# igrega348/energy-equiv-lattice-gnn

Hardware: AMD Instinct MI355X
Metric: lattice-graphs/s (fwd+bwd), 4-layer EnergyEquivGNN, ~1k nodes/~4k edges, 1/2/4/8 GPU (higher is better)
Workload: dtype f32

## Files before the change

energy-equiv-lattice-gnn_amd/gnn/_lib.py:

```python
from __future__ import annotations

import ctypes
import os
from typing import Dict, Optional, Tuple

import torch

LIB_PATH = os.environ.get("EELG_LIB") or os.path.join(os.path.dirname(os.path.abspath(__file__)),
                                                      "libeelg.so")

_P = ctypes.c_void_p
_I = ctypes.c_int
_F = ctypes.c_float
_D = ctypes.c_double
_LL = ctypes.c_longlong

_SIGS = {
    "eelg_version": ([], ctypes.c_char_p),
    "eelg_last_error": ([], ctypes.c_char_p),
    "eelg_tp_find": ([ctypes.c_char_p], _I),
    "eelg_tp_info": ([_I, _P, _P], _I),
    "eelg_sc_find": ([ctypes.c_char_p], _I),
    "eelg_sc_info": ([_I, _P, _P], _I),
    "eelg_sc_outputs": ([_I, _P], _I),
# ... 29 lines not shown
    "eelg_cgc_fwd": ([_P, _P, _P, _P, _P, _P, _I, _I, _P, _P], _I),
    "eelg_cgc_bwd": ([_P, _P, _P, _P, _P, _P, _I, _I, _P, _P, _P, _P], _I),
    "eelg_cgc_fwd_ef": ([_P, _P, _P, _P, _P, _P, _P, _P, _I, _I, _P, _P], _I),
    "eelg_cgc_fwd_ef_res": ([_P] * 6 + [_P, _I, _I, _P, _P, _P], _I),
    "eelg_cgc_bwd_ef": ([_P, _P, _P, _P, _P, _P, _P, _P, _I, _I, _P, _P, _P, _P, _P], _I),
    "eelg_cgc_bwd_ef_parts": ([_I], _I),
    "eelg_nnconv_fwd": ([_P, _P, _P, _P, _P, _I, _I, _P, _P], _I),
    "eelg_nnconv_bwd_edge": ([_P, _P, _P, _P, _P, _P, _I, _I, _P, _P, _P, _P], _I),
    "eelg_nnconv_bwd_w_parts": ([_I, _I], _I),
    "eelg_nnconv_bwd_w": ([_P, _P, _P, _P, _P, _P, _I, _I, _P, _P, _P], _I),
    "eelg_csr_spmm": ([_P, _P, _P, _I, _P, _I, _I, _I, _P, _I, _I, _P], _I),
    "eelg_sc_fwd": ([_I, _P, _P, _I, _I, _P, _P], _I),
    "eelg_sc_bwd_x": ([_I, _P, _P, _P, _I, _I, _P, _P], _I),
    "eelg_sc_bwd_x_cm": ([_I, _P, _P, _P, _I, _I, _P, _P, _P, _P], _I),
    "eelg_sc_bwd_coef": ([_I, _P, _P, _I, _I, _I, _P, _P], _I),
    "eelg_sc_bwd_coef_parts": ([_I, _I, _I], _I),
    "eelg_sc_cmajor": ([_I, _I, _P, _I, _I, _P, _P], _I),
    "eelg_scg_fwd": ([_P, _P, _P, _I, _P, _I, _I, _P, _I, _P], _I),
    "eelg_scg_bwd_x": ([_P, _P, _P, _I, _P, _I, _P, _I, _I, _P, _P], _I),
    "eelg_scg_bwd_coef": ([_P, _P, _P, _I, _P, _I, _P, _I, _I, _P, _P], _I),
    "eelg_linear_fwd": ([_P, _I, _P, _P, _I, _P, _I, _P, _P], _I),
    "eelg_linear_fwd_res": ([_P, _I, _P, _P, _P, _I, _P, _I, _P, _P], _I),
    "eelg_linear_bwd_w": ([_P, _I, _P, _I, _I, _I, _P, _I, _I, _P, _P], _I),
    "eelg_linear_bwd_w_x6": ([_P, _I, _P, _I, _I, _I, _I, _I, _P, _P], _I),
    "eelg_radial_plan": ([_I, _I, _P, _P], _I),
    "eelg_linear_pack_size": ([_P], ctypes.c_longlong),
    "eelg_linear_pack": ([_P, _P, _P, _P], _I),
    "eelg_linear_fwd_pk": ([_P, _I, _P, _P, _P, _I, _P, _I, _P, _P], _I),
    "eelg_split_bf16x3": ([_P, ctypes.c_longlong, _P, _P], _I),
    "eelg_sum_rows_work": ([_I, ctypes.c_longlong], ctypes.c_longlong),
    "eelg_sum_rows": ([_P, ctypes.c_longlong, _I, ctypes.c_longlong, ctypes.c_float, _P, _P,
                       ctypes.c_longlong, _P], _I),
    "eelg_radial_fwd": ([_P, _I, _P, _P, _I, _P, _P, _P], _I),
    "eelg_radial_bwd_chain": ([_P, _I, _I, _P, _P, _P, _P, _P, _P, _P, _P], _I),
    "eelg_radial_bwd_chain_rows": ([_P, _I, _I, _P, _I, _P, _P, _P, _P, _P, _P, _P, _P, _P], _I),
    "eelg_radial_bwd": ([_P, _I, _I, _P, _P, _P, _P, _P, _P, _P, _P], _I),
    "eelg_tp_bwd_sh": ([_I, _P, _P, _P, _P, _P, _I, _P, _F, _P, _P], _I),
    "eelg_radial_bwd_x": ([_P, _I, _P, _P, _P, _P], _I),
    "eelg_radial_bwd_gh": ([_P, _I, _I, _P, _P, _P, _P], _I),
    "eelg_edge_embed_bwd": ([_P, _P, _P, _P, _P, _I, _I, _I, _F, _F, _P, _I, _P, _P, _P, _P], _I),
    "eelg_batch_assemble": ([_P, _P, _P, _I, _I, _I, _P, _P], _I),
    "eelg_mandel_rotate": ([_P, _I, _P, _P, _I, _P, _P], _I),
    "eelg_stiffness_metrics": ([_P, _P, _P, _I, _I, _F, _P, _P], _I),
    "eelg_elastic_props": ([_P, _P, _I, _I, _P, _P, _P, _P], _I),
    "eelg_elastic_props_bwd": ([_P, _P, _P, _P, _P, _P, _I, _I, _P, _P], _I),
    "eelg_transverse_props": ([_P, _P, _I, _I, _P, _P, _P, _P, _P, _P], _I),
    "eelg_transverse_props_bwd": ([_P, _P, _P, _P, _P, _P, _I, _I, _P, _P], _I),
    "eelg_stiffness_loss": ([_P, _P, _I, _I, _F, _P, _P, _P], _I),
    "eelg_sqnorm_parts": ([_LL], _I),
    "eelg_grad_sqnorm": ([_P, _LL, _P, _P], _I),
    "eelg_adamw_flat": ([_P, _P, _P, _P, _P, _LL, _P, _D, _D, _D, _D, _D, _D, _I, _P, _P, _P], _I),
    "eelg_strut_volume": ([_P] * 9 + [_I, _I, _I, _P, _P], _I),
    "eelg_design_step": ([_P] * 16 + [_I, _I, _I] + [_F] * 6 + [_I, _P, _P, _P], _I),
}

LIN_MAXSRC, LIN_MAXSLOT, LINW_MAXINS = 4, 8, 8


class LinSrc(ctypes.Structure):
    _fields_ = [("x_off", _I), ("k", _I), ("w_off", _I), ("ldk", _I), ("ldj", _I), ("alpha", _F)]


class LinSlot(ctypes.Structure):
    _fields_ = [("y_off", _I), ("n_out", _I), ("d", _I), ("bias_off", _I), ("n_src", _I),
                ("src", LinSrc * LIN_MAXSRC), ("r_off", _I)]


class LinDesc(ctypes.Structure):
    _fields_ = [("n_slots", _I), ("max_jt", _I), ("max_rows", _I), ("res_row", _I),
                ("slot", LinSlot * LIN_MAXSLOT)]


class LinWIns(ctypes.Structure):
    _fields_ = [("x_off", _I), ("k", _I), ("g_off", _I), ("n_out", _I), ("d", _I), ("w_off", _I),
                ("alpha", _F), ("ldw", _I)]


class LinWDesc(ctypes.Structure):
    _fields_ = [("n_ins", _I), ("max_jt", _I), ("max_ut", _I), ("max_rows", _I),
                ("ins", LinWIns * LINW_MAXINS)]

BATCH_MAXW = 64
METRICS_COLS = 16
ELASTIC_COLS = 12
TRANSVERSE_COLS = 7
TRANSVERSE_DIR_COLS = 5
OPTIM_STATE_COLS = 4
DESIGN_THREADS = 256


class BatchSrc(ctypes.Structure):
    _fields_ = [(k, _P) for k in ("positions", "node_attrs", "rowend", "srowend", "sender", "receiver",
                                  "shifts", "edge_attr", "perm", "sperm")] + \
               [(k, _I) for k in ("node_w", "edge_w", "total_nodes", "total_edges")]


class BatchOut(ctypes.Structure):
    _fields_ = [(k, _P) for k in ("positions", "node_attrs", "batch", "ptr", "rowptr", "srowptr",
                                  "edge_index", "shifts", "edge_attr", "perm", "sperm", "sender",
                                  "receiver")]


RADIAL_MAXH = 3
GATE_MAXBLK = 8
CGC_MAXD = 256
NNC_WIDTHS = (32, 64)
GATE_MAXGATED = 2048
GATE_MAXGATES = 512


class GateDesc(ctypes.Structure):
    _fields_ = [("n_scal", _I), ("n_gates", _I), ("n_blk", _I), ("pad", _I),
                ("blk_mul", _I * GATE_MAXBLK), ("blk_dim", _I * GATE_MAXBLK)]


SCG_MAXD = 25
SCG_CHUNK = 256


class ScgDesc(ctypes.Structure):
    _fields_ = [("D", _I), ("Dout", _I), ("mul", _I), ("nterms", _I),
                ("xb", _I * SCG_MAXD), ("xs", _I * SCG_MAXD), ("ob", _I * SCG_MAXD),
                ("os", _I * SCG_MAXD), ("orow", _I * (SCG_MAXD + 1))]


class RadialDesc(ctypes.Structure):
    _fields_ = [("n_feat", _I), ("hidden", _I), ("n_hidden", _I), ("n_out", _I),
                ("w", _P * RADIAL_MAXH), ("b", _P * RADIAL_MAXH)]


EXPORTED_SYMBOLS = tuple(_SIGS)

_lib = None


class EELGError(RuntimeError):
    pass


def load() -> ctypes.CDLL:
    global _lib
# ... 143 lines not shown
```

energy-equiv-lattice-gnn_amd/gnn/model.py:

```python
from __future__ import annotations

import os
from argparse import Namespace
from typing import Any, Dict

import torch

from . import ops
from .blocks import (Cart_4_to_Mandel, GeneralNonLinearReadoutBlock, MACELayer, PositiveLayer,
                     Spherical_to_Cartesian, as_csr)
from .irreps import Irreps
from .o3 import Linear


def storage_dtype(params: Namespace) -> torch.dtype:
    name = str(getattr(params, "storage_dtype", "float32")).replace("torch.", "")
    table = {"float32": torch.float32, "fp32": torch.float32, "bfloat16": torch.bfloat16,
             "bf16": torch.bfloat16}
    if name not in table:
        raise ValueError(f"storage_dtype {name!r}: expected 'float32' or 'bfloat16'")
    return table[name]


RADIAL_AHEAD_OF_LAYER1 = os.environ.get("EELG_RADIAL_BEFORE_L1", "1") != "0"
# ... 114 lines not shown
    def _radial_weights_ahead(self, edge_feats, csr=None, edge_sh=None):
        geom = torch.is_grad_enabled() and edge_feats.requires_grad
        if geom or not (ops.OVERLAP and edge_feats.is_cuda):
            return [None] * self.num_interactions, [None] * self.num_interactions
        main = torch.cuda.current_stream(edge_feats.device)
        side = ops.side_stream(edge_feats.device)
        side.wait_stream(main)
        edge_feats.record_stream(side)
        ws, evs = [], []
        with torch.cuda.stream(side):
            for layer in self.layers:
                smap = layer.interaction.strut_map(csr, edge_feats, edge_sh) if csr is not None else None
                w = layer.interaction.radial_weights(edge_feats, smap)
                ev = torch.cuda.Event()
                ev.record(side)
                ws.append(w)
                evs.append(ev)
        for w in ws:
            self._main_stream_weight(w).record_stream(main)
        return ws, evs

    @staticmethod
    def _main_stream_weight(w):
        return w.w if isinstance(w, ops.StrutWeights) else w

    def _coefficients_ahead(self, device) -> None:
        if not (ops.OVERLAP and COEF_AHEAD and device.type == "cuda"):
            return
        main = torch.cuda.current_stream(device)
        side = ops.side_stream(device, 1)
        side.wait_stream(main)
        for i, layer in enumerate(self.layers):
            layer.product.symmetric_contractions.coefficients_ahead(
                side, live=self.live_pruned and i == self.num_interactions - 1)

    def forward(self, edge_index, node_ft, edge_sh, edge_feats, batch_idx, num_graphs: int):
        csr, edge_sh, edge_feats = as_csr(edge_index, node_ft.shape[0], edge_sh, edge_feats)
        ws, evs = self._radial_weights_ahead(edge_feats, csr, edge_sh)
        self._coefficients_ahead(node_ft.device)

        def run(i, h, residual=None):
            if evs[i] is not None:
                torch.cuda.current_stream(h.device).wait_event(evs[i])
            live = self.live_pruned and i == self.num_interactions - 1
            return self.layers[i](h, csr, edge_sh, edge_feats, tp_weights=ws[i], residual=residual,
                                  live=live)

        node_ft = run(0, node_ft)
        if RADIAL_AHEAD_OF_LAYER1 and evs[-1] is not None:
            torch.cuda.current_stream(node_ft.device).wait_event(evs[-1])
        for i in range(1, self.num_interactions):
            node_ft = run(i, node_ft, residual=node_ft)
        out = self.nonlin_readout(node_ft, live=self.live_pruned)
        graph_ft = ops.graph_pool(out, batch_idx, num_graphs, self.global_reduction)
        stiff = self.sph_to_cart(self.linear(graph_ft, live=self.live_pruned))
        return self.positive_layer(self.cart_to_Mandel(stiff))


class _Embed1(torch.autograd.Function):

    @staticmethod
    def forward(ctx, attrs, weight, bias):
        ctx.save_for_backward(attrs)
        ctx.has_bias = bias is not None
        w = weight[:, 0]
        return torch.addcmul(bias, attrs, w) if bias is not None else attrs * w

    @staticmethod
    def backward(ctx, gy):
        from . import ops
        (attrs,) = ctx.saved_tensors
        gy = ops._f32(gy).contiguous()
        gw = ops.sum_rows(gy * attrs).unsqueeze(1) if ctx.needs_input_grad[1] else None
        gb = ops.sum_rows(gy) if ctx.has_bias and ctx.needs_input_grad[2] else None
        return None, gw, gb


def _embed(lin: torch.nn.Linear, attrs: torch.Tensor) -> torch.Tensor:
    if lin.in_features != 1:
        return lin(attrs)
    if attrs.is_cuda and not attrs.requires_grad:
        return _Embed1.apply(attrs, lin.weight, lin.bias)
    return torch.addcmul(lin.bias, attrs, lin.weight[:, 0]) if lin.bias is not None \
        else attrs * lin.weight[:, 0]


def _geometry_key(batch, n_edges: int):
    ts = [getattr(batch, k, None) for k in ("positions", "shifts", "edge_attr")]
    if not all(torch.is_tensor(t) for t in ts) or any(t.requires_grad for t in ts):
        return None
    pos, shifts, radius = ts
    if radius.numel() != n_edges or tuple(shifts.shape) != (n_edges, 3) or pos.dim() != 2 or pos.shape[1] != 3:
        return None
    return tuple((t.data_ptr(), t._version, tuple(t.shape), str(t.device)) for t in ts)


class EnergyEquivGNN(torch.nn.Module):
    def __init__(self, params: Namespace, *args: Any, **kwargs: Any) -> None:
        super().__init__(*args, **kwargs)
        self.params = params
        hidden = Irreps(params.hidden_irreps)
        self.node_ft_embedding = torch.nn.Linear(1, hidden.count("0e"))
        self.number_of_edge_basis = params.num_edge_bases
        self.max_edge_radius = params.max_edge_radius
        self.lmax = params.lmax
        self.stiffness_head = GNN_Head(params)

    @staticmethod
    def edge_graph(batch, strut: bool = True, build: bool = True) -> ops.EdgeCSR:
        n = batch.node_attrs.shape[0]
        ei = batch.edge_index
        dev = ei.device
        key = (ei.data_ptr(), ei._version, tuple(ei.shape), n, str(dev))
        csr = getattr(batch, "_eelg_csr", None)
        if csr is None or getattr(batch, "_eelg_csr_key", None) != key:
            pre = getattr(batch, "csr", None)
            if isinstance(pre, dict) and torch.is_tensor(pre.get("perm")):
                csr = ops.EdgeCSR.from_dict({k: (v.to(dev) if torch.is_tensor(v) else v)
                                             for k, v in pre.items()}, n)
            else:
                csr = ops.EdgeCSR.build(batch.edge_index, n)
            try:
                batch._eelg_csr = csr
                batch._eelg_csr_key = key
            except AttributeError:
                pass
        geo_key = _geometry_key(batch, csr.num_edges) if strut and ops.STRUT_WEIGHTS else None
        if geo_key is None:
            return csr
        if csr.strut is not None and getattr(csr, "_strut_key", None) != geo_key:
            csr.strut = None
        if csr.strut is None and build:
            csr.strut = ops.build_strut_map(batch.positions, csr.sender, csr.receiver,
                                            batch.shifts[csr.perm], batch.edge_attr[csr.perm].reshape(-1))
            csr._strut_key = geo_key
        return csr

    def forward(self, batch) -> Dict[str, torch.Tensor]:
        dev = batch.positions.device
        if dev.type != "cuda":
            raise RuntimeError("the EnergyEquivGNN hot path runs only on a HIP device "
                               "(got a CPU batch); move the model and batch to 'cuda'")
        with torch.cuda.device(dev):
            return self._forward(batch)

    def _forward(self, batch) -> Dict[str, torch.Tensor]:
        csr = self.edge_graph(batch, build=False)
        node_ft = _embed(self.node_ft_embedding, batch.node_attrs)
        geom = torch.is_grad_enabled() and (batch.positions.requires_grad or batch.shifts.requires_grad
                                            or batch.edge_attr.requires_grad)
        if geom and storage_dtype(self.params) != torch.float32:
            raise NotImplementedError(
                "geometry gradients (positions / shifts / edge_attr requiring grad) are built for "
                "fp32 storage only, not storage_dtype='bfloat16'")
        shifts = ops.permute_rows(batch.shifts, csr.perm)
        radius = ops.permute_rows(batch.edge_attr, csr.perm).reshape(-1)
        edge_sh, edge_feats = ops.edge_embed(batch.positions, csr, shifts, radius, self.lmax,
                                             self.number_of_edge_basis, 0.6, self.max_edge_radius)
        c = self.stiffness_head(csr, node_ft, edge_sh, edge_feats, batch.batch, batch.num_graphs)
        return {"stiffness": c}
```

energy-equiv-lattice-gnn_amd/gnn/ops.py:

```python
from __future__ import annotations

import contextlib
import ctypes
import math
import os
import weakref
from dataclasses import dataclass
from typing import Dict, Optional

import torch

from . import _lib


KernelTimer, TIMER, _launch = _lib.KernelTimer, _lib.TIMER, _lib.launch

OVERLAP = os.environ.get("EELG_OVERLAP", "1") != "0"
LIVE_OUT = os.environ.get("EELG_LIVE_OUT", "1") != "0"
SC_CMAJOR_ON_SIDE = os.environ.get("EELG_SC_CMAJOR_SIDE", "0") != "0"
SC_COEF_ON_SIDE = os.environ.get("EELG_SC_COEF_SIDE", "1") != "0"
RADIAL_CHAIN = os.environ.get("EELG_RADIAL_CHAIN", "1") != "0"
_TBS = os.environ.get("EELG_TP_BWD_SENDER", "0")
TP_BWD_SENDER = None if _TBS == "auto" else _TBS != "0"
TP_BWD_SPOS = os.environ.get("EELG_TP_BWD_SPOS", "0") != "0"
# ... 47 lines not shown
    def rep_rows(self, feats: torch.Tensor) -> torch.Tensor:
        memo = getattr(self, "_rep_rows", None)
        if memo is not None and memo[0]() is feats and memo[1] == feats._version:
            return memo[2]
        rows = feats[self.rep]
        self._rep_rows = (weakref.ref(feats), feats._version, rows)
        return rows


def _key_bits(v: torch.Tensor) -> torch.Tensor:
    return (v + 0.0).contiguous().view(torch.int32).to(torch.int64)


def build_strut_map(pos: torch.Tensor, sender: torch.Tensor, receiver: torch.Tensor,
                    shifts_sorted: torch.Tensor, radius_sorted: torch.Tensor) -> StrutMap:
    e = int(sender.shape[0])
    dev = sender.device
    ar = torch.arange(e, device=dev)
    if e == 0:
        z = torch.zeros(0, device=dev, dtype=torch.int64)
        return StrutMap(z, z.to(torch.int32), z, 0)
    s, r = sender.long(), receiver.long()
    pos = pos.detach().to(torch.float32)
    vec = (pos[r] - pos[s]) + shifts_sorted.detach().to(torch.float32)
    rad = _key_bits(radius_sorted.detach().to(torch.float32).reshape(e, 1))
    fwd = torch.cat([s[:, None], r[:, None], _key_bits(vec), rad], 1)
    rev = torch.cat([r[:, None], s[:, None], _key_bits(-vec), rad], 1)
    _, inv = torch.unique(torch.cat([fwd, rev]), dim=0, return_inverse=True)
    kf, kr = inv[:e], inv[e:]
    nk = int(inv.max()) + 1
    cnt = torch.zeros(nk, device=dev, dtype=torch.int64).index_add_(0, kf, torch.ones_like(kf))
    owner = torch.full((nk,), -1, device=dev, dtype=torch.int64)
    owner[kf] = ar
    cand = owner[kr]
    ok = (cnt[kf] == 1) & (cnt[kr] == 1) & (cand >= 0)
    partner = torch.where(ok, cand, ar)
    is_rep = partner >= ar
    rep = torch.nonzero(is_rep).reshape(-1)
    row_of = torch.cumsum(is_rep.to(torch.int64), 0) - 1
    row = row_of[torch.minimum(partner, ar)].to(torch.int32)
    return StrutMap(partner, row.contiguous(), rep, int(rep.shape[0]))


@dataclass
class EdgeCSR:
    perm: torch.Tensor
    sender: torch.Tensor
    receiver: torch.Tensor
    rowptr: torch.Tensor
    sperm: torch.Tensor
    srowptr: torch.Tensor
    num_nodes: int
    strut: Optional[StrutMap] = None

    @property
    def num_edges(self) -> int:
        return int(self.sender.shape[0])

    def sender_pos(self) -> torch.Tensor:
        sp = getattr(self, "_spos", None)
        if sp is None:
            sp = torch.empty_like(self.sperm)
            sp[self.sperm.long()] = torch.arange(self.sperm.shape[0], device=self.sperm.device,
                                                 dtype=self.sperm.dtype)
            self._spos = sp
        return sp

    @staticmethod
    def from_dict(d: Dict, num_nodes: int) -> "EdgeCSR":
        return EdgeCSR(d["perm"], d["sender"], d["receiver"], d["rowptr"], d["sperm"],
                       d["srowptr"], num_nodes)

    @staticmethod
    def build(edge_index: torch.Tensor, num_nodes: int) -> "EdgeCSR":
        from .data import build_edge_csr
        return EdgeCSR.from_dict(build_edge_csr(edge_index, num_nodes), num_nodes)


def edge_embed(pos, csr: EdgeCSR, shifts_sorted, radius_sorted, lmax: int, nb: int,
               len_end: float, rad_end: float):
    _require_device(pos, shifts_sorted, radius_sorted)
    if torch.is_grad_enabled() and (pos.requires_grad or shifts_sorted.requires_grad
                                    or radius_sorted.requires_grad):
        return _EdgeEmbed.apply(pos, shifts_sorted, radius_sorted, csr, lmax, nb, float(len_end),
                                float(rad_end))
    return _edge_embed_fwd(pos, csr, shifts_sorted, radius_sorted, lmax, nb, len_end, rad_end)


def _edge_embed_fwd(pos, csr: EdgeCSR, shifts_sorted, radius_sorted, lmax: int, nb: int,
                    len_end: float, rad_end: float):
    e = csr.num_edges
    nsh = (lmax + 1) ** 2
    sh = torch.empty(e, sh_row_stride(nsh), device=pos.device, dtype=torch.float32)
    feats = torch.empty(e, 2 * nb, device=pos.device, dtype=torch.float32)
    _launch("edge_embed", _lib.load().eelg_edge_embed, _f32(pos), csr.sender, csr.receiver,
            _f32(shifts_sorted), _f32(radius_sorted), e, lmax, nb, float(len_end), float(rad_end),
            sh, feats, on=sh)
    return sh[:, :nsh], feats


class _EdgeEmbed(torch.autograd.Function):

    @staticmethod
    def forward(ctx, pos, shifts_sorted, radius_sorted, csr: EdgeCSR, lmax, nb, len_end, rad_end):
        pos, shifts_sorted, radius_sorted = _f32(pos), _f32(shifts_sorted), _f32(radius_sorted)
        ctx.save_for_backward(pos, shifts_sorted, radius_sorted)
# ... 64 lines not shown
def padded_sh(sh: torch.Tensor) -> torch.Tensor:
    nsh = sh.shape[1]
    nshp = sh_row_stride(nsh)
    if (sh.dtype == torch.float32 and sh.stride() == (nshp, 1) and sh.storage_offset() == 0
            and sh.untyped_storage().nbytes() >= sh.shape[0] * nshp * 4):
        return sh
    out = torch.zeros(sh.shape[0], nshp, device=sh.device, dtype=torch.float32)
    out[:, :nsh] = sh
    return out[:, :nsh]


def segment_sum_csr(src, rowptr, n_rows: int, idx=None, row_scale=None, scale: float = 1.0):
    _require_device(src)
    bf = src.dtype == torch.bfloat16
    src = src.contiguous() if bf else _f32(src)
    width = src[0].numel() if src.shape[0] > 0 else int(torch.tensor(src.shape[1:]).prod())
    out = torch.empty((n_rows,) + tuple(src.shape[1:]), device=src.device, dtype=torch.float32)
    lib = _lib.load()
    fn = lib.eelg_segment_sum_csr_bf16 if bf else lib.eelg_segment_sum_csr
    _launch("segment_sum_csr", fn, src, rowptr, idx, row_scale, float(scale), n_rows, int(width), out,
            on=out)
    return out


def segment_sum_long(src: torch.Tensor, rowptr: torch.Tensor, n_rows: int,
                     row_scale: Optional[torch.Tensor] = None, scale: float = 1.0) -> torch.Tensor:
    _require_device(src)
    src = _f32(src)
    width = src.shape[1]
    n_split = max(1, min(64, -(-2048 // max(n_rows, 1))))
    work = torch.empty(n_rows, n_split, width, device=src.device, dtype=torch.float32)
    out = torch.empty(n_rows, width, device=src.device, dtype=torch.float32)
    _launch("segment_sum_split", _lib.load().eelg_segment_sum_split, src, rowptr, None, row_scale,
            float(scale), n_rows, width, n_split, work, out, on=out, timed="segment_sum_split")
    return out


class _SegmentMean(torch.autograd.Function):

    @staticmethod
    def forward(ctx, src, ptr32, batch, inv_cnt):
        ctx.save_for_backward(batch, inv_cnt)
        n_rows = ptr32.shape[0] - 1
        if src.shape[0] >= 64 * max(n_rows, 1):
            return segment_sum_long(src, ptr32, n_rows, row_scale=inv_cnt)
        return segment_sum_csr(src, ptr32, n_rows, row_scale=inv_cnt)

    @staticmethod
    def backward(ctx, g):
        batch, inv_cnt = ctx.saved_tensors
        return (g * inv_cnt[:, None])[batch], None, None, None


def graph_pool(src, batch, num_graphs: int, reduce: str = "mean"):
    _require_device(src)
    bounds = torch.arange(num_graphs + 1, device=batch.device, dtype=batch.dtype)
    ptr = torch.searchsorted(batch, bounds).to(torch.int32)
    cnt = (ptr[1:] - ptr[:-1]).to(torch.int64)
    if reduce == "mean":
        inv = 1.0 / cnt.clamp_min(1).to(torch.float32)
    elif reduce in ("sum", "add"):
        inv = torch.ones(num_graphs, device=src.device, dtype=torch.float32)
    elif reduce in ("max", "min", "mul"):
        return segment_pool_order(src, ptr, num_graphs, reduce)
    else:
        raise ValueError(f"global_reduction {reduce!r} not supported "
                         "(torch_scatter reduces: sum, add, mean, max, min, mul)")
    return _SegmentMean.apply(src, ptr, batch, inv)


_ORDER_OPS = {"max": 0, "min": 1, "mul": 2}


class _SegmentOrder(torch.autograd.Function):

    @staticmethod
    def forward(ctx, src, rowptr, n_rows: int, op: int, covered: bool):
        src = _f32(src)
        width = src.shape[1]
        out = torch.empty(n_rows, width, device=src.device, dtype=torch.float32)
        arg = (torch.empty(n_rows, width, device=src.device, dtype=torch.int32)
               if op != _ORDER_OPS["mul"] else None)
        _launch("segment_order", _lib.load().eelg_segment_order, src, rowptr, n_rows, width, op, out,
                arg, on=out)
        ctx.save_for_backward(src, rowptr, arg)
        ctx.n_rows, ctx.op, ctx.covered = n_rows, op, covered
        return out

    @staticmethod
    def backward(ctx, g):
        src, rowptr, arg = ctx.saved_tensors
        g = _f32(g)
        gs = torch.empty_like(src) if ctx.covered else torch.zeros_like(src)
        _launch("segment_order_bwd", _lib.load().eelg_segment_order_bwd, src, rowptr, arg, g,
                ctx.n_rows, src.shape[1], ctx.op, gs, on=gs)
        return gs, None, None, None, None


def segment_order(src, rowptr32, n_rows: int, reduce: str, covered: bool = False):
    _require_device(src)
    if reduce not in _ORDER_OPS:
        raise ValueError(f"segment_order: reduce {reduce!r} (max, min, mul)")
    return _SegmentOrder.apply(src, rowptr32, n_rows, _ORDER_OPS[reduce], covered)


def segment_pool_order(src, ptr32, num_graphs: int, reduce: str):
    return segment_order(src, ptr32, num_graphs, reduce)


PNA_FUSED = os.environ.get("EELG_PNA_FUSED", "1") != "0"
PNA_EPS = 1e-5


# ... 926 lines not shown
        g = _f32(g)
        sp, mul = ctx.sp, ctx.mul
        nt, nk = sp.shape
        a, t = sp.on(g.device)
        gt = g.t().contiguous()
        gw = torch.empty(nk, mul, device=g.device, dtype=torch.float32)
        _spmm(t, nk, gt, mul, 1, mul, gw, mul, 1)
        return gw, None, None


def symcon_coefficients(w: torch.Tensor, sp: SparseRows, ld: Optional[int] = None) -> torch.Tensor:
    return _SymConCoef.apply(w, sp, sp.shape[0] if ld is None else ld)


LOSS_FUSED = os.environ.get("EELG_LOSS_FUSED", "1") != "0"


class _StiffnessLoss(torch.autograd.Function):
    @staticmethod
    def forward(ctx, pred, target, grad_scale: float):
        _require_device(pred, target)
        nb = int(target.shape[0])
        p2 = _f32(pred).reshape(nb, -1)
        t2 = _f32(target).reshape(nb, -1)
        n = int(t2.shape[1])
        out = torch.empty(2, device=pred.device, dtype=torch.float32)
        grad = torch.empty_like(p2)
        with torch.cuda.device(pred.device):
            _launch("stiffness_loss", _lib.load().eelg_stiffness_loss, p2, t2, nb, n,
                    float(grad_scale), out, grad, on=pred, timed="stiffness_loss")
        ctx.save_for_backward(grad)
        ctx.shape = pred.shape
        loss, mean = out[0], out[1]
        ctx.mark_non_differentiable(mean)
        return loss, mean

    @staticmethod
    def backward(ctx, g_loss, g_mean):
        (grad,) = ctx.saved_tensors
        return (grad * g_loss).view(ctx.shape), None, None


def stiffness_loss_fused(pred: torch.Tensor, target: torch.Tensor, grad_scale: float = 1.0):
    if tuple(pred.shape) != tuple(target.shape) or pred.dim() < 2:
        raise ValueError(f"stiffness_loss_fused: pred {tuple(pred.shape)}, target {tuple(target.shape)}")
    if LOSS_FUSED and pred.is_cuda:
        return _StiffnessLoss.apply(pred, target.detach(), float(grad_scale))
    dims = tuple(range(1, target.dim()))
    per_graph = torch.nn.functional.mse_loss(pred, target, reduction="none").mean(dim=dims)
    loss = 100 * (per_graph / target.pow(2).mean(dim=dims)).mean()
    if grad_scale != 1.0:
        loss = loss.detach() + (loss - loss.detach()) * grad_scale
    return loss, per_graph.detach().mean()
```

include/eelg.h:

```cpp
#ifndef EELG_H
#define EELG_H

#include <stdint.h>

#ifdef __cplusplus
extern "C" {
#endif

const char* eelg_version(void);
const char* eelg_last_error(void);

int eelg_tp_find(const char* name);
int eelg_tp_info(int cfg, int* info7, uint64_t* sig);
int eelg_sc_find(const char* name);
int eelg_sc_info(int cfg, int* info8, uint64_t* sig);
int eelg_sc_outputs(int cfg, int* ls8);
int eelg_sc_find_outputs(int cfg, const int* ls, int n_ls);

int eelg_edge_embed(const float* pos, const int* sender, const int* receiver, const float* shifts,
                    const float* radius, int n_edges, int lmax, int nb, float len_end,
                    float rad_end, float* sh, float* feats, void* stream);

int eelg_tp_fwd(int cfg, const float* x, const float* sh, const float* w, const int* sender,
                const int* rowptr, int n_nodes, float inv_norm, float* agg, void* stream);
// ... 237 lines not shown
  int64_t* edge_index; float* shifts; float* edge_attr; int64_t* perm; int* sperm; int* sender;
  int* receiver;
} eelg_batch_out;
int eelg_batch_assemble(const eelg_batch_src* src, const int* table, const float* rot, int n_graphs,
                        int n_nodes, int n_edges, const eelg_batch_out* out, void* stream);

int eelg_mandel_rotate(const float* src, int n_src, const int* sel, const float* rot, int n_graphs,
                       float* out, void* stream);

#define EELG_METRICS_COLS 16
int eelg_stiffness_metrics(const float* pred, const float* target, const float* dirs, int n_graphs,
                           int n_dirs, float scale, float* out, void* stream);

#define EELG_ELASTIC_COLS 12
int eelg_elastic_props(const float* c, const float* dirs, int n_graphs, int n_dirs, float* props,
                       float* e_dir, float* s, void* stream);
int eelg_elastic_props_bwd(const float* s, const float* dirs, const float* e_dir, const float* props,
                           const float* g_props, const float* g_e_dir, int n_graphs, int n_dirs,
                           float* g_c, void* stream);

#define EELG_TRANSVERSE_COLS 7
#define EELG_TRANSVERSE_DIR_COLS 5
int eelg_transverse_props(const float* c, const float* dirs, int n_graphs, int n_dirs, float* props,
                          float* t_dir, int* arg, float* n_ext, double* s, void* stream);
int eelg_transverse_props_bwd(const double* s, const float* dirs, const float* props, const int* arg,
                              const float* g_props, const float* g_t_dir, int n_graphs, int n_dirs,
                              float* g_c, void* stream);

#define EELG_SQNORM_CHUNK 8192
#define EELG_SQNORM_MAXPARTS 1024
#define EELG_OPTIM_STATE_COLS 4
int eelg_stiffness_loss(const float* pred, const float* target, int n_graphs, int n, float grad_scale,
                        float* out, float* grad, void* stream);
int eelg_sqnorm_parts(long long numel);
int eelg_grad_sqnorm(const float* grad, long long numel, float* partials, void* stream);
int eelg_adamw_flat(float* p, float* m, float* v, float* vmax, float* grad, long long numel,
                    const float* partials, double lr, double beta1, double beta2, double eps,
                    double weight_decay, double max_norm, int amsgrad, const int* state_in, int* state_out,
                    void* stream);

#define EELG_DESIGN_THREADS 256
int eelg_strut_volume(const float* pos, const float* r, const float* shifts, const int* send,
                      const int* recv, const int* node_ptr, const int* edge_ptr,
                      const int* node_ptr_host, const int* edge_ptr_host, int n_graphs, int n_nodes,
                      int n_edges, float* vol, void* stream);
int eelg_design_step(const float* g_pos, const float* g_r, float* pos, float* r, const float* pos0,
                     float* m_pos, float* m_r, const int* partner, const int* node_ptr,
                     const int* edge_ptr, const int* node_ptr_host, const int* edge_ptr_host,
                     const float* shifts, const int* send, const int* recv, const float* v0,
                     int n_graphs, int n_nodes, int n_edges, float step_r, float step_pos, float beta,
                     float r_min, float r_max, float move_limit, int keep_volume, float* vol, int* flag,
                     void* stream);

#ifdef __cplusplus
}
#endif
#endif
```

Measured before the change: 2342.

## Fuse stiffness head (linear, sph-to-cart, Mandel, positive map) into one kernel

Adds a HIP kernel that, per graph, applies the final equivariant linear, the spherical-to-Cartesian projection, the Mandel mapping and the positive matrix function in one block, with a matching backward kernel that computes per-graph input, weight and bias gradients and sums them afterwards. This replaces a chain of small per-op launches and autograd nodes at the end of the model. It also caches the graph-pool segment bounds on the CSR object so searchsorted is not redone every step. In exchange, the kernels do their arithmetic in double precision with one 64-thread block per graph, and the backward writes per-graph weight-gradient rows that need an extra reduction.

```diff
diff --git a/energy-equiv-lattice-gnn_amd/csrc/eelg_head.hip b/energy-equiv-lattice-gnn_amd/csrc/eelg_head.hip
--- /dev/null
+++ b/energy-equiv-lattice-gnn_amd/csrc/eelg_head.hip
@@ -0,0 +1,250 @@
+#include <hip/hip_runtime.h>
+#include <stdint.h>
+
+#include "../../include/eelg.h"
+#include "eelg_internal.h"
+
+#define HEAD_THREADS 64
+#define HEAD_Y 21
+#define HEAD_CART 81
+#define HEAD_C 36
+
+template <typename TI, typename TO>
+__device__ __forceinline__ void head_linear(const eelg_lin_desc& desc, const TI* __restrict__ in,
+                                            const float* __restrict__ w, const float* __restrict__ bias,
+                                            TO* __restrict__ out) {
+  int base = 0;
+  for (int s = 0; s < desc.n_slots; ++s) {
+    const eelg_lin_slot& sl = desc.slot[s];
+    const int d = sl.d, cols = sl.n_out * d;
+    for (int c = (int)threadIdx.x - base; c < cols; c += HEAD_THREADS) {
+      if (c < 0) continue;
+      const int j = c / d, m = c - j * d;
+      double acc = 0.0;
+      for (int t = 0; t < sl.n_src; ++t) {
+        const eelg_lin_src& src = sl.src[t];
+        const TI* __restrict__ xi = in + src.x_off + m;
+        const float* __restrict__ wj = w + src.w_off + (size_t)j * src.ldj;
+        for (int k = 0; k < src.k; ++k) acc = fma((double)xi[k * d], (double)(wj[(size_t)k * src.ldk] * src.alpha), acc);
+      }
+      if (bias && sl.bias_off >= 0) acc += (double)bias[sl.bias_off + j];
+      out[sl.y_off + c] = (TO)acc;
+    }
+    base = (base + cols) % HEAD_THREADS;
+  }
+}
+
+__device__ __forceinline__ double head_base(double a, int idx, int pos) {
+  const double eye = (idx / 6 == idx % 6) ? 1.0 : 0.0;
+  if (pos == EELG_HEAD_TRUNC_EXP_2) return eye + a / 2.0;
+  if (pos == EELG_HEAD_TRUNC_EXP_4) return eye + a / 4.0;
+  return a;
+}
+
+__device__ __forceinline__ double head_square(const double* m, int i, int j) {
+  double acc = 0.0;
+#pragma unroll
+  for (int k = 0; k < 6; ++k) acc = fma(m[i * 6 + k], m[k * 6 + j], acc);
+  return acc;
+}
+
+__device__ __forceinline__ double head_square_bwd(const double* g, const double* m, int i, int j) {
+  double acc = 0.0;
+#pragma unroll
+  for (int k = 0; k < 6; ++k) acc = fma(g[i * 6 + k], m[j * 6 + k], acc);
+#pragma unroll
+  for (int k = 0; k < 6; ++k) acc = fma(m[k * 6 + i], g[k * 6 + j], acc);
+  return acc;
+}
+
+__device__ __forceinline__ bool head_squares(int pos) { return pos != EELG_HEAD_NONE; }
+__device__ __forceinline__ bool head_fourth(int pos) {
+  return pos == EELG_HEAD_POWER_4 || pos == EELG_HEAD_TRUNC_EXP_4;
+}
+
+__global__ __launch_bounds__(HEAD_THREADS) void head_fwd_kernel(
+    const float* __restrict__ x, int x_row, const float* __restrict__ w, const float* __restrict__ bias,
+    eelg_lin_desc desc, const float* __restrict__ q, const float* __restrict__ map, int pos,
+    float* __restrict__ c_out, float* __restrict__ a_out) {
+  __shared__ double s_y[HEAD_Y], s_z[HEAD_CART], s_m[HEAD_C], s_s[HEAD_C];
+  const int b = blockIdx.x, tid = threadIdx.x;
+  if (tid < HEAD_Y) s_y[tid] = 0.0;
+  __syncthreads();
+  head_linear(desc, x + (size_t)b * x_row, w, bias, s_y);
+  __syncthreads();
+  for (int r = tid; r < HEAD_CART; r += HEAD_THREADS) {
+    double acc = 0.0;
+#pragma unroll
+    for (int i = 0; i < HEAD_Y; ++i) acc = fma(s_y[i], (double)q[i * HEAD_CART + r], acc);
+    s_z[r] = acc;
+  }
+  __syncthreads();
+  double a = 0.0;
+  if (tid < HEAD_C) {
+    for (int r = 0; r < HEAD_CART; ++r) a = fma(s_z[r], (double)map[r * HEAD_C + tid], a);
+    a_out[(size_t)b * HEAD_C + tid] = (float)a;
+    s_m[tid] = head_base(a, tid, pos);
+  }
+  __syncthreads();
+  double c = a;
+  if (head_squares(pos)) {
+    if (tid < HEAD_C) c = head_square(s_m, tid / 6, tid % 6);
+    if (head_fourth(pos)) {
+      if (tid < HEAD_C) s_s[tid] = c;
+      __syncthreads();
+      if (tid < HEAD_C) c = head_square(s_s, tid / 6, tid % 6);
+    }
+  }
+  if (tid < HEAD_C) c_out[(size_t)b * HEAD_C + tid] = (float)c;
+}
+
+__global__ __launch_bounds__(HEAD_THREADS) void head_bwd_kernel(
+    const float* __restrict__ g_c, const float* __restrict__ a_in, const float* __restrict__ x, int x_row,
+    const float* __restrict__ w, eelg_lin_desc fdesc, eelg_lin_desc xdesc, eelg_linw_desc wdesc,
+    const float* __restrict__ q, const float* __restrict__ map, int pos, int n_w, int n_b,
+    float* __restrict__ g_x, int gx_row, float* __restrict__ g_wb) {
+  extern __shared__ float s_w[];
+  __shared__ double s_y[HEAD_Y], s_z[HEAD_CART], s_m[HEAD_C], s_s[HEAD_C], s_g[HEAD_C], s_t[HEAD_C];
+  const int b = blockIdx.x, tid = threadIdx.x;
+  const int i6 = tid / 6, j6 = tid % 6;
+  for (int e = tid; e < n_w + n_b; e += HEAD_THREADS) s_w[e] = 0.f;
+  if (tid < HEAD_C) {
+    s_m[tid] = head_base((double)a_in[(size_t)b * HEAD_C + tid], tid, pos);
+    s_g[tid] = (double)g_c[(size_t)b * HEAD_C + tid];
+  }
+  __syncthreads();
+  if (head_squares(pos)) {
+    if (head_fourth(pos)) {
+      if (tid < HEAD_C) s_s[tid] = head_square(s_m, i6, j6);
+      __syncthreads();
+      if (tid < HEAD_C) s_t[tid] = head_square_bwd(s_g, s_s, i6, j6);
+      __syncthreads();
+      if (tid < HEAD_C) s_g[tid] = s_t[tid];
+      __syncthreads();
+    }
+    double ga = 0.0;
+    if (tid < HEAD_C) {
+      ga = head_square_bwd(s_g, s_m, i6, j6);
+      if (pos == EELG_HEAD_TRUNC_EXP_2) ga = ga / 2.0;
+      if (pos == EELG_HEAD_TRUNC_EXP_4) ga = ga / 4.0;
+    }
+    __syncthreads();
+    if (tid < HEAD_C) s_g[tid] = ga;
+    __syncthreads();
+  }
+  for (int r = tid; r < HEAD_CART; r += HEAD_THREADS) {
+    double acc = 0.0;
+#pragma unroll
+    for (int c = 0; c < HEAD_C; ++c) acc = fma((double)map[r * HEAD_C + c], s_g[c], acc);
+    s_z[r] = acc;
+  }
+  __syncthreads();
+  if (tid < HEAD_Y) {
+    double acc = 0.0;
+    for (int r = 0; r < HEAD_CART; ++r) acc = fma((double)q[tid * HEAD_CART + r], s_z[r], acc);
+    s_y[tid] = acc;
+  }
+  __syncthreads();
+  head_linear(xdesc, s_y, w, nullptr, g_x + (size_t)b * gx_row);
+  const float* __restrict__ xb = x + (size_t)b * x_row;
+  for (int t = 0; t < wdesc.n_ins; ++t) {
+    const eelg_linw_ins& in = wdesc.ins[t];
+    const int ldw = in.ldw ? in.ldw : in.n_out;
+    for (int e = tid; e < in.k * in.n_out; e += HEAD_THREADS) {
+      const int u = e / in.n_out, j = e - u * in.n_out;
+      double acc = 0.0;
+      for (int m = 0; m < in.d; ++m)
+        acc = fma((double)xb[in.x_off + u * in.d + m], s_y[in.g_off + j * in.d + m], acc);
+      s_w[in.w_off + u * ldw + j] = (float)(acc * (double)in.alpha);
+    }
+  }
+  for (int s = 0; s < fdesc.n_slots; ++s) {
+    const eelg_lin_slot& sl = fdesc.slot[s];
+    if (sl.bias_off < 0) continue;
+    for (int j = tid; j < sl.n_out; j += HEAD_THREADS) s_w[n_w + sl.bias_off + j] = (float)s_y[sl.y_off + j];
+  }
+  __syncthreads();
+  for (int e = tid; e < n_w + n_b; e += HEAD_THREADS) g_wb[(size_t)b * (n_w + n_b) + e] = s_w[e];
+}
+
+static int head_desc_check(const eelg_lin_desc* desc, int in_len, int out_len, int n_w, int n_b,
+                           bool covers, const char* what) {
+  if (!desc || desc->n_slots <= 0 || desc->n_slots > EELG_LIN_MAXSLOT)
+    return eelg_fail(-2, "%s: bad descriptor", what);
+  long long covered = 0;
+  for (int s = 0; s < desc->n_slots; ++s) {
+    const eelg_lin_slot& sl = desc->slot[s];
+    if (sl.n_src < 0 || sl.n_src > EELG_LIN_MAXSRC || sl.d <= 0 || sl.n_out <= 0 || sl.y_off < 0 ||
+        (long long)sl.y_off + (long long)sl.n_out * sl.d > out_len)
+      return eelg_fail(-2, "%s: slot %d leaves the output row of %d", what, s, out_len);
+    covered += (long long)sl.n_out * sl.d;
+    if (sl.bias_off >= 0 && (sl.d != 1 || sl.bias_off + sl.n_out > n_b))
+      return eelg_fail(-2, "%s: slot %d: bias on a non-scalar slot or past %d biases", what, s, n_b);
+    for (int t = 0; t < sl.n_src; ++t) {
+      const eelg_lin_src& src = sl.src[t];
+      if (src.k <= 0 || src.x_off < 0 || (long long)src.x_off + (long long)src.k * sl.d > in_len)
+        return eelg_fail(-2, "%s: slot %d source %d leaves the input row of %d", what, s, t, in_len);
+      if (src.w_off < 0 || src.ldk < 0 || src.ldj < 0 ||
+          (long long)src.w_off + (long long)(src.k - 1) * src.ldk + (long long)(sl.n_out - 1) * src.ldj >= n_w)
+        return eelg_fail(-2, "%s: slot %d source %d leaves the %d weights", what, s, t, n_w);
+    }
+  }
+  if (covers && covered != out_len)
+    return eelg_fail(-2, "%s: the slots cover %lld of the %d output columns", what, covered, out_len);
+  return 0;
+}
+
+static int head_pos_check(int pos, const char* what) {
+  if (pos < EELG_HEAD_NONE || pos > EELG_HEAD_TRUNC_EXP_4)
+    return eelg_fail(-2, "%s: positive function %d (EELG_HEAD_NONE .. EELG_HEAD_TRUNC_EXP_4)", what, pos);
+  return 0;
+}
+
+extern "C" {
+
+int eelg_head_fwd(const float* x, int x_row, int n_feat, const float* w, int n_w, const float* bias, int n_b,
+                  const eelg_lin_desc* desc, const float* q_flat, const float* map, int pos, int n_graphs,
+                  float* c, float* a, void* stream) {
+  if (n_graphs <= 0) return eelg_fail(-2, "head_fwd: %d graphs (at least 1)", n_graphs);
+  if (!x || !w || !q_flat || !map || !c || !a || (n_b > 0 && !bias))
+    return eelg_fail(-2, "head_fwd: null pointer (x, w, bias, q_flat, map, c, a)");
+  if (n_feat <= 0 || x_row < n_feat || n_w <= 0 || n_b < 0)
+    return eelg_fail(-2, "head_fwd: bad sizes (n_feat %d, x_row %d, n_w %d, n_b %d)", n_feat, x_row, n_w, n_b);
+  if (int rc = head_pos_check(pos, "head_fwd")) return rc;
+  if (int rc = head_desc_check(desc, n_feat, HEAD_Y, n_w, n_b, false, "head_fwd")) return rc;
+  hipLaunchKernelGGL(head_fwd_kernel, dim3((unsigned)n_graphs), dim3(HEAD_THREADS), 0, (hipStream_t)stream, x,
+                     x_row, w, n_b > 0 ? bias : nullptr, *desc, q_flat, map, pos, c, a);
+  return eelg_check_launch("head_fwd");
+}
+
+int eelg_head_bwd(const float* g_c, const float* a, const float* x, int x_row, int n_feat, const float* w,
+                  int n_w, int n_b, const eelg_lin_desc* fwd_desc, const eelg_lin_desc* bx_desc,
+                  const eelg_linw_desc* bw_desc, const float* q_flat, const float* map, int pos, int n_graphs,
+                  float* g_x, float* g_wb, void* stream) {
+  if (n_graphs <= 0) return eelg_fail(-2, "head_bwd: %d graphs (at least 1)", n_graphs);
+  if (!g_c || !a || !x || !w || !q_flat || !map || !g_x || !g_wb)
+    return eelg_fail(-2, "head_bwd: null pointer (g_c, a, x, w, q_flat, map, g_x, g_wb)");
+  if (n_feat <= 0 || x_row < n_feat || n_w <= 0 || n_b < 0 || n_w + n_b > EELG_HEAD_MAXW)
+    return eelg_fail(-2, "head_bwd: bad sizes (n_feat %d, x_row %d, n_w %d, n_b %d; n_w + n_b <= %d)", n_feat,
+                     x_row, n_w, n_b, EELG_HEAD_MAXW);
+  if (int rc = head_pos_check(pos, "head_bwd")) return rc;
+  if (int rc = head_desc_check(fwd_desc, n_feat, HEAD_Y, n_w, n_b, false, "head_bwd (forward descriptor)")) return rc;
+  if (int rc = head_desc_check(bx_desc, HEAD_Y, n_feat, n_w, 0, true, "head_bwd (grad-x descriptor)")) return rc;
+  if (!bw_desc || bw_desc->n_ins < 0 || bw_desc->n_ins > EELG_LINW_MAXINS)
+    return eelg_fail(-2, "head_bwd: bad grad-W descriptor");
+  for (int t = 0; t < bw_desc->n_ins; ++t) {
+    const eelg_linw_ins& in = bw_desc->ins[t];
+    const long long ldw = in.ldw ? in.ldw : in.n_out;
+    if (in.k <= 0 || in.n_out <= 0 || in.d <= 0 || in.x_off < 0 || in.g_off < 0 || in.w_off < 0 || in.ldw < 0 ||
+        ldw < in.n_out || (long long)in.x_off + (long long)in.k * in.d > n_feat ||
+        (long long)in.g_off + (long long)in.n_out * in.d > HEAD_Y ||
+        (long long)in.w_off + (long long)(in.k - 1) * ldw + in.n_out > n_w)
+      return eelg_fail(-2, "head_bwd: grad-W instruction %d leaves its arrays", t);
+  }
+  hipLaunchKernelGGL(head_bwd_kernel, dim3((unsigned)n_graphs), dim3(HEAD_THREADS),
+                     (size_t)(n_w + n_b) * sizeof(float), (hipStream_t)stream, g_c, a, x, x_row, w, *fwd_desc,
+                     *bx_desc, *bw_desc, q_flat, map, pos, n_w, n_b, g_x, n_feat, g_wb);
+  return eelg_check_launch("head_bwd");
+}
+
+}
diff --git a/energy-equiv-lattice-gnn_amd/gnn/_lib.py b/energy-equiv-lattice-gnn_amd/gnn/_lib.py
--- a/energy-equiv-lattice-gnn_amd/gnn/_lib.py
+++ b/energy-equiv-lattice-gnn_amd/gnn/_lib.py
@@ -105,6 +105,8 @@
     "eelg_adamw_flat": ([_P, _P, _P, _P, _P, _LL, _P, _D, _D, _D, _D, _D, _D, _I, _P, _P, _P], _I),
     "eelg_strut_volume": ([_P] * 9 + [_I, _I, _I, _P, _P], _I),
     "eelg_design_step": ([_P] * 16 + [_I, _I, _I] + [_F] * 6 + [_I, _P, _P, _P], _I),
+    "eelg_head_fwd": ([_P, _I, _I, _P, _I, _P, _I, _P, _P, _P, _I, _I, _P, _P, _P], _I),
+    "eelg_head_bwd": ([_P, _P, _P, _I, _I, _P, _I, _I, _P, _P, _P, _P, _P, _I, _I, _P, _P, _P], _I),
 }
 
 LIN_MAXSRC, LIN_MAXSLOT, LINW_MAXINS = 4, 8, 8
@@ -140,6 +142,7 @@
 TRANSVERSE_DIR_COLS = 5
 OPTIM_STATE_COLS = 4
 DESIGN_THREADS = 256
+HEAD_MAXW = 8192
 
 
 class BatchSrc(ctypes.Structure):
diff --git a/energy-equiv-lattice-gnn_amd/gnn/model.py b/energy-equiv-lattice-gnn_amd/gnn/model.py
--- a/energy-equiv-lattice-gnn_amd/gnn/model.py
+++ b/energy-equiv-lattice-gnn_amd/gnn/model.py
@@ -190,7 +190,25 @@
         for i in range(1, self.num_interactions):
             node_ft = run(i, node_ft, residual=node_ft)
         out = self.nonlin_readout(node_ft, live=self.live_pruned)
-        graph_ft = ops.graph_pool(out, batch_idx, num_graphs, self.global_reduction)
+        graph_ft = ops.graph_pool(out, batch_idx, num_graphs, self.global_reduction,
+                                  bounds=ops.pool_bounds_of(csr, batch_idx, num_graphs))
+        return self.stiffness_from_pooled(graph_ft)
+
+    def _head_fusable(self, graph_ft) -> bool:
+        lin = self.linear
+        ts = (graph_ft, lin.weight, lin.bias, self.sph_to_cart.Q_flat, self.cart_to_Mandel.map)
+        return bool(ops.HEAD_FUSED and self.params.positive_function in ops.HEAD_POSITIVE
+                    and type(lin) is Linear and lin.irreps_out.dim == ops.HEAD_OUT
+                    and graph_ft.dim() == 2 and graph_ft.shape[0] > 0
+                    and all(t is None or (t.is_cuda and t.dtype == torch.float32
+                                          and t.device == graph_ft.device) for t in ts))
+
+    def stiffness_from_pooled(self, graph_ft):
+        if self._head_fusable(graph_ft):
+            lin = self.linear
+            k = lin.live if (self.live_pruned and lin.live is not None) else lin
+            return ops.stiffness_head(graph_ft, k, lin.weight, lin.bias, self.sph_to_cart.Q_flat,
+                                      self.cart_to_Mandel.map, self.params.positive_function)
         stiff = self.sph_to_cart(self.linear(graph_ft, live=self.live_pruned))
         return self.positive_layer(self.cart_to_Mandel(stiff))
 
@@ -263,6 +281,12 @@
                 batch._eelg_csr_key = key
             except AttributeError:
                 pass
+        bvec, ng = getattr(batch, "batch", None), getattr(batch, "num_graphs", None)
+        if torch.is_tensor(bvec) and isinstance(ng, int) and bvec.device == dev:
+            if ops.pool_bounds_of(csr, bvec, ng) is None:
+                csr.pool = ops.pool_bounds(bvec, ng)
+        else:
+            csr.pool = None
         geo_key = _geometry_key(batch, csr.num_edges) if strut and ops.STRUT_WEIGHTS else None
         if geo_key is None:
             return csr
diff --git a/energy-equiv-lattice-gnn_amd/gnn/ops.py b/energy-equiv-lattice-gnn_amd/gnn/ops.py
--- a/energy-equiv-lattice-gnn_amd/gnn/ops.py
+++ b/energy-equiv-lattice-gnn_amd/gnn/ops.py
@@ -123,6 +123,7 @@
     srowptr: torch.Tensor
     num_nodes: int
     strut: Optional[StrutMap] = None
+    pool: Optional["PoolBounds"] = None
 
     @property
     def num_edges(self) -> int:
@@ -293,13 +294,40 @@
         return (g * inv_cnt[:, None])[batch], None, None, None
 
 
-def graph_pool(src, batch, num_graphs: int, reduce: str = "mean"):
-    _require_device(src)
+@dataclass
+class PoolBounds:
+    ptr: torch.Tensor
+    cnt: torch.Tensor
+    inv: torch.Tensor
+    key: tuple
+
+
+def pool_bounds_key(batch: torch.Tensor, num_graphs: int) -> tuple:
+    return (batch.data_ptr(), batch._version, tuple(batch.shape), int(num_graphs), str(batch.device))
+
+
+def pool_bounds(batch: torch.Tensor, num_graphs: int) -> PoolBounds:
     bounds = torch.arange(num_graphs + 1, device=batch.device, dtype=batch.dtype)
     ptr = torch.searchsorted(batch, bounds).to(torch.int32)
     cnt = (ptr[1:] - ptr[:-1]).to(torch.int64)
+    inv = 1.0 / cnt.clamp_min(1).to(torch.float32)
+    return PoolBounds(ptr, cnt, inv, pool_bounds_key(batch, num_graphs))
+
+
+def pool_bounds_of(csr, batch: torch.Tensor, num_graphs: int) -> Optional[PoolBounds]:
+    pb = getattr(csr, "pool", None)
+    if pb is None or pb.key != pool_bounds_key(batch, num_graphs):
+        return None
+    return pb
+
+
+def graph_pool(src, batch, num_graphs: int, reduce: str = "mean", bounds: Optional[PoolBounds] = None):
+    _require_device(src)
+    if bounds is None:
+        bounds = pool_bounds(batch, num_graphs)
+    ptr, cnt = bounds.ptr, bounds.cnt
     if reduce == "mean":
-        inv = 1.0 / cnt.clamp_min(1).to(torch.float32)
+        inv = bounds.inv
     elif reduce in ("sum", "add"):
         inv = torch.ones(num_graphs, device=src.device, dtype=torch.float32)
     elif reduce in ("max", "min", "mul"):
@@ -1332,3 +1360,75 @@
     if grad_scale != 1.0:
         loss = loss.detach() + (loss - loss.detach()) * grad_scale
     return loss, per_graph.detach().mean()
+
+
+HEAD_FUSED = os.environ.get("EELG_HEAD_FUSED", "1") != "0"
+HEAD_POSITIVE = {"none": 0, "matrix_power_2": 1, "matrix_power_4": 2, "matrix_trunc_exp_2": 3,
+                 "matrix_trunc_exp_4": 4}
+HEAD_OUT = 21
+
+
+def _head_sizes(k, weight, bias):
+    n_w, n_b = int(weight.numel()), 0 if bias is None else int(bias.numel())
+    if k._out_dim != HEAD_OUT or n_w + n_b > _lib.HEAD_MAXW:
+        raise ValueError(f"stiffness_head: a linear onto {k._out_dim} columns with {n_w} + {n_b} "
+                         f"parameters (expected {HEAD_OUT} columns, at most {_lib.HEAD_MAXW})")
+    return n_w, n_b
+
+
+def _head_fwd(x, k, weight, bias, q_flat, cmap, pos: int, c=None, a=None):
+    nb = int(x.shape[0])
+    n_w, n_b = _head_sizes(k, weight, bias)
+    c = torch.empty(nb, 36, device=x.device, dtype=torch.float32) if c is None else c
+    a = torch.empty(nb, 36, device=x.device, dtype=torch.float32) if a is None else a
+    _launch("head_fwd", _lib.load().eelg_head_fwd, x, k._in_dim, k._in_dim, weight, n_w, bias, n_b,
+            k._fwd_desc, q_flat, cmap, pos, nb, c, a, on=x, timed="head_fwd")
+    return c, a
+
+
+def _head_bwd(gc, a, x, k, weight, bias, q_flat, cmap, pos: int, gx=None, gwb=None):
+    nb = int(x.shape[0])
+    n_w, n_b = _head_sizes(k, weight, bias)
+    gx = torch.empty(nb, k._in_dim, device=x.device, dtype=torch.float32) if gx is None else gx
+    gwb = torch.empty(nb, n_w + n_b, device=x.device, dtype=torch.float32) if gwb is None else gwb
+    _launch("head_bwd", _lib.load().eelg_head_bwd, gc, a, x, k._in_dim, k._in_dim, weight, n_w, n_b,
+            k._fwd_desc, k._bx_desc, k._bw_desc, q_flat, cmap, pos, nb, gx, gwb, on=x, timed="head_bwd")
+    return gx, gwb
+
+
+class _StiffnessHead(torch.autograd.Function):
+    @staticmethod
+    def forward(ctx, x, weight, bias, q_flat, cmap, k, pos: int):
+        x = _f32(x)
+        weight, q_flat, cmap = _f32(weight), _f32(q_flat), _f32(cmap)
+        bias = None if bias is None else _f32(bias)
+        with torch.cuda.device(x.device):
+            c, a = _head_fwd(x, k, weight, bias, q_flat, cmap, pos)
+        ctx.save_for_backward(x, weight, bias, q_flat, cmap, a)
+        ctx.k, ctx.pos = k, pos
+        return c.view(-1, 6, 6)
+
+    @staticmethod
+    def backward(ctx, gc):
+        x, weight, bias, q_flat, cmap, a = ctx.saved_tensors
+        gc = _f32(gc).reshape(-1, 36)
+        with torch.cuda.device(x.device):
+            gx, gwb = _head_bwd(gc, a, x, ctx.k, weight, bias, q_flat, cmap, ctx.pos)
+            gsum = sum_rows(gwb)
+        n_w = weight.numel()
+        return (gx if ctx.needs_input_grad[0] else None, gsum[:n_w] if ctx.needs_input_grad[1] else None,
+                gsum[n_w:] if (bias is not None and ctx.needs_input_grad[2]) else None, None, None, None, None)
+
+
+def stiffness_head(graph_ft: torch.Tensor, k, weight: torch.Tensor, bias: Optional[torch.Tensor],
+                   q_flat: torch.Tensor, cmap: torch.Tensor, positive_function: str) -> torch.Tensor:
+    _require_device(graph_ft, weight, bias, q_flat, cmap)
+    if positive_function not in HEAD_POSITIVE:
+        raise ValueError(f"stiffness_head: positive function {positive_function!r} is not covered "
+                         f"({sorted(HEAD_POSITIVE)})")
+    if graph_ft.dim() != 2 or graph_ft.shape[1] != k._in_dim:
+        raise ValueError(f"stiffness_head expects [B, {k._in_dim}], got {tuple(graph_ft.shape)}")
+    if tuple(q_flat.shape) != (HEAD_OUT, 81) or tuple(cmap.shape) != (81, 36):
+        raise ValueError(f"stiffness_head: Q_flat {tuple(q_flat.shape)}, map {tuple(cmap.shape)}: "
+                         "expected [21, 81] and [81, 36]")
+    return _StiffnessHead.apply(graph_ft, weight, bias, q_flat, cmap, k, HEAD_POSITIVE[positive_function])
diff --git a/include/eelg.h b/include/eelg.h
--- a/include/eelg.h
+++ b/include/eelg.h
@@ -313,6 +313,20 @@
                      float r_min, float r_max, float move_limit, int keep_volume, float* vol, int* flag,
                      void* stream);
 
+#define EELG_HEAD_NONE 0
+#define EELG_HEAD_POWER_2 1
+#define EELG_HEAD_POWER_4 2
+#define EELG_HEAD_TRUNC_EXP_2 3
+#define EELG_HEAD_TRUNC_EXP_4 4
+#define EELG_HEAD_MAXW 8192
+int eelg_head_fwd(const float* x, int x_row, int n_feat, const float* w, int n_w, const float* bias, int n_b,
+                  const eelg_lin_desc* desc, const float* q_flat, const float* map, int pos, int n_graphs,
+                  float* c, float* a, void* stream);
+int eelg_head_bwd(const float* g_c, const float* a, const float* x, int x_row, int n_feat, const float* w,
+                  int n_w, int n_b, const eelg_lin_desc* fwd_desc, const eelg_lin_desc* bx_desc,
+                  const eelg_linw_desc* bw_desc, const float* q_flat, const float* map, int pos, int n_graphs,
+                  float* g_x, float* g_wb, void* stream);
+
 #ifdef __cplusplus
 }
 #endif
```

After: 2274. 0.971x the previous value.
